# roahmlab/koopman-realizations

Hardware: AMD Instinct MI355X
Metric: EDMD snapshot-pairs/sec (bilinear fit, 3-link arm, poly-3) (higher is better)
Workload: dtype f64

## Files before the change

### koopman-realizations_amd/csrc/kp_context.hip

```cpp
#include <algorithm>
#include <cmath>
#include <cstring>
#include <mutex>

#include "kp_internal.h"

static std::mutex g_err_mu;
static std::string g_err;

void kp_set_global_error(const std::string& s) {
  std::lock_guard<std::mutex> l(g_err_mu);
  g_err = s;
}

void* kp_ctx::workspace(int slot, size_t bytes) {
  if (ws_bytes[slot] >= bytes && ws[slot]) return ws[slot];
  if (ws[slot]) (void)hipFree(ws[slot]);
  ws[slot] = nullptr;
  ws_bytes[slot] = 0;
  size_t want = bytes + bytes / 4 + 256;
  if (hipMalloc(&ws[slot], want) != hipSuccess) return nullptr;
  ws_bytes[slot] = want;
  return ws[slot];
}
// ... 50 lines not shown
  (void)kp_flush_grams(c);
  (void)kp_comm_destroy(c);
  (void)hipSetDevice(c->device);
  kp_stage_destroy(c);
  (void)hipStreamSynchronize(c->stream);
  if (c->stream2) (void)hipStreamSynchronize(c->stream2);
  for (int i = 0; i < 21; ++i)
    if (c->ws[i]) (void)hipFree(c->ws[i]);
  if (c->sticky_info) (void)hipFree(c->sticky_info);
  if (c->pin_small) (void)hipHostFree(c->pin_small);
  if (c->pin_scratch) (void)hipHostFree(c->pin_scratch);
  if (c->ev_gram_done) (void)hipEventDestroy(c->ev_gram_done);
  if (c->ev_pad_done) (void)hipEventDestroy(c->ev_pad_done);
  if (c->ev_pad_done2) (void)hipEventDestroy(c->ev_pad_done2);
  if (c->ev_main_done) (void)hipEventDestroy(c->ev_main_done);
  if (c->ev_solve0) (void)hipEventDestroy(c->ev_solve0);
  if (c->ev_solve1) (void)hipEventDestroy(c->ev_solve1);
  if (c->stream2) (void)hipStreamDestroy(c->stream2);
  if (c->Kres) (void)hipFree(c->Kres);
  if (c->GC) (void)hipFree(c->GC);
  for (int i = 0; i < 6; ++i)
    if (c->evp[i]) (void)hipEventDestroy(c->evp[i]);
  for (int i = 0; i < 2 * 64; ++i)
    if (c->ring[i]) (void)hipEventDestroy(c->ring[i]);
  for (int i = 0; i < 64; ++i)
    if (c->ring_red[i]) (void)hipEventDestroy(c->ring_red[i]);
  (void)hipEventDestroy(c->ev0);
  (void)hipEventDestroy(c->ev1);
  (void)hipStreamDestroy(c->stream);
  kp_traj_pool_free(c);
  kp_host_free_all(c);
  delete c;
  return KP_OK;
}

extern "C" int kp_device_count(int* count) {
  if (!count) return KP_ERR_ARG;
  int n = 0;
  if (hipGetDeviceCount(&n) != hipSuccess) {
    (void)hipGetLastError();
    n = 0;
  }
  *count = n;
  return KP_OK;
}

extern "C" const char* kp_last_error(const kp_ctx* c) {
  if (c) return c->err.c_str();
  std::lock_guard<std::mutex> l(g_err_mu);
  static thread_local std::string copy;
  copy = g_err;
  return copy.c_str();
}

extern "C" int kp_device_info(const kp_ctx* c, char* name, int name_len, int* num_cu, int64_t* hbm) {
  if (!c) return KP_ERR_ARG;
  if (name && name_len > 0) {
    std::strncpy(name, c->name.c_str(), (size_t)name_len - 1);
    name[name_len - 1] = 0;
  }
  if (num_cu) *num_cu = c->num_cu;
  if (hbm) *hbm = c->hbm_bytes;
  return KP_OK;
}

void* kp_pinned_scratch(kp_ctx* ctx, size_t bytes) {
  if (ctx->pin_scratch_bytes >= bytes) return ctx->pin_scratch;
  if (ctx->pin_scratch) {
    (void)hipStreamSynchronize(ctx->stream);
    (void)hipHostFree(ctx->pin_scratch);
  }
  ctx->pin_scratch = nullptr;
  ctx->pin_scratch_bytes = 0;
  const size_t cap = (bytes + 4095) & ~(size_t)4095;
  if (hipHostMalloc(&ctx->pin_scratch, cap, hipHostMallocDefault) != hipSuccess) {
    ctx->pin_scratch = nullptr;
    return nullptr;
  }
  ctx->pin_scratch_bytes = cap;
  return ctx->pin_scratch;
}

extern "C" int kp_timer_get(const kp_ctx* c, int which, double* ms) {
  if (!c || !ms || which < 0 || which >= 18) return KP_ERR_ARG;
  *ms = c->timers[which];
  return KP_OK;
}

extern "C" void* kp_stream(const kp_ctx* c) { return c ? (void*)c->stream : nullptr; }


static int upload(kp_ctx* ctx, void** dst, const void* src, size_t bytes) {
  *dst = nullptr;
  if (bytes == 0) return KP_OK;
  KP_HIP(ctx, hipMalloc(dst, bytes));
  KP_HIP(ctx, hipMemcpy(*dst, src, bytes, hipMemcpyHostToDevice));
  return KP_OK;
}

extern "C" int kp_basis_desc_dims(const kp_basis_desc* d, int* nvars_out, int* nfull_out, int* N_out, int* W_out) {
  if (!d || d->nzeta < 1 || d->m < 0 || d->model_type < 0 || d->model_type > 2 || d->n_blocks < 0 ||
      (d->n_blocks && (!d->block_type || !d->block_count)))
    return KP_ERR_ARG;
  const int nvars = d->nzeta + (d->model_type == KP_MODEL_NONLINEAR ? d->m : 0);
  double nf = nvars + 1.0;
  for (int b = 0; b < d->n_blocks; ++b) {
    const int c = d->block_count[b];
    if (c < 0) return KP_ERR_ARG;
    switch (d->block_type[b]) {
      case KP_BLOCK_POLY: case KP_BLOCK_HERMITE: case KP_BLOCK_FOURIER_SPARSER: case KP_BLOCK_GAUSSIAN: nf += c; break;
      case KP_BLOCK_FOURIER: nf += std::pow((double)(2 * c + 1), (double)nvars) - 1.0; break;
      default: return KP_ERR_ARG;
    }
    if (nf > 1e6) return KP_ERR_ARG;
  }
  const int nfull = (int)std::llround(nf);
  const int N = d->k_pcs > 0 ? d->k_pcs + nvars + 1 : nfull;
  if (nvars_out) *nvars_out = nvars;
  if (nfull_out) *nfull_out = nfull;
  if (N_out) *N_out = N;
  if (W_out) *W_out = d->model_type == KP_MODEL_BILINEAR ? N * (d->m + 1) : d->model_type == KP_MODEL_LINEAR ? N + d->m : N;
  return KP_OK;
}

extern "C" int kp_basis_create(kp_ctx* ctx, const kp_basis_desc* d, kp_basis** out) {
  if (!ctx || !d || !out) return KP_ERR_ARG;
  *out = nullptr;
  KP_HIP(ctx, hipSetDevice(ctx->device));
  if (d->model_type < 0 || d->model_type > 2) return ctx->fail(KP_ERR_ARG, "kp_basis_create: model_type");
  if (d->nzeta < 1 || d->m < 0) return ctx->fail(KP_ERR_ARG, "kp_basis_create: nzeta/m");
  int nvars = d->nzeta + (d->model_type == KP_MODEL_NONLINEAR ? d->m : 0);
  if (nvars > KP_MAX_VARS) return ctx->fail(KP_ERR_ARG, "kp_basis_create: too many variables (max 32)");
  std::vector<ColDesc> cols;
  for (int i = 0; i < nvars; ++i) cols.push_back({COL_VAR, i, 0, 0});
  int n_mono = 0, n_gauss = 0, max_deg = 1, fourier_deg = 0;
  for (int b = 0; b < d->n_blocks; ++b) {
    int cnt = d->block_count[b];
    if (cnt < 0) return ctx->fail(KP_ERR_ARG, "kp_basis_create: negative block count");
    switch (d->block_type[b]) {
      case KP_BLOCK_POLY:
        if (cnt && !d->poly_exps) return ctx->fail(KP_ERR_ARG, "kp_basis_create: poly_exps is NULL");
        for (int i = 0; i < cnt; ++i) {
          int deg = 0;
          for (int v = 0; v < nvars; ++v) deg += d->poly_exps[(size_t)(n_mono + i) * nvars + v];
          if (deg > max_deg) max_deg = deg;
          uint32_t pk[2] = {0, 0};
          if (nvars <= 8)
            for (int v = 0; v < nvars; ++v) pk[v >> 2] |= (uint32_t)d->poly_exps[(size_t)(n_mono + i) * nvars + v] << (8 * (v & 3));
          cols.push_back({COL_MONO, n_mono + i, (int32_t)pk[0], (int32_t)pk[1]});
        }
        n_mono += cnt;
        break;
      case KP_BLOCK_FOURIER: {
        if (cnt < 1) return ctx->fail(KP_ERR_ARG, "kp_basis_create: fourier degree < 1");
        double nf = std::pow((double)(2 * cnt + 1), (double)nvars);
        if (nf > 1e6) return ctx->fail(KP_ERR_ARG, "kp_basis_create: fourier block too large");
        int total = (int)std::llround(nf);
        for (int i = 1; i < total; ++i) {
          uint32_t pk = 0;
          if (nvars <= 8 && 2 * cnt + 1 <= 16) {
            int idx = i;
            for (int v = nvars - 1; v >= 0; --v) {
              pk |= (uint32_t)(idx % (2 * cnt + 1)) << (4 * v);
              idx /= 2 * cnt + 1;
            }
          }
          cols.push_back({COL_FOURIER, i, cnt, (int32_t)pk});
// ... 380 lines not shown
```

### koopman-realizations_amd/csrc/kp_fit.hip

```cpp
#include <cmath>
#include <cstdlib>

#include <vector>
#include <algorithm>
#include <cstring>

#include "kp_internal.h"

typedef double double4_t __attribute__((ext_vector_type(4)));
extern "C" int kp_synchronize(kp_ctx* ctx);

__global__ __launch_bounds__(256) void kp_pad_kernel(const double* __restrict__ G, const double* __restrict__ C, int W, int ncols, int n, int ncp,
                                                     double* __restrict__ Gp, double* __restrict__ Cp, size_t gc_stride) {
  const int i = blockIdx.x * 256 + threadIdx.x, jj = blockIdx.y;
  if (i >= n) return;
  G += blockIdx.z * gc_stride; C += blockIdx.z * gc_stride; Gp += blockIdx.z * (size_t)n * n; Cp += blockIdx.z * (size_t)n * ncp;
  if (jj < n) {
    Gp[(size_t)jj * n + i] = (i < W && jj < W) ? G[(size_t)jj * W + i] : (i == jj ? 1.0 : 0.0);
  } else {
    const int j = jj - n;
    Cp[(size_t)j * n + i] = (i < W && j < ncols) ? C[(size_t)j * W + i] : 0.0;
  }
}

__global__ __launch_bounds__(256) void kp_unpad_kernel(const double* __restrict__ Xp, int n, int W, int ncols, double* __restrict__ K, int ncp, int k_first, int k_cap) {
  const int i = blockIdx.x * 256 + threadIdx.x, j = blockIdx.y;
  if (i >= W) return;
  Xp += blockIdx.z * (size_t)n * ncp;
  if (k_cap > 0) K += (size_t)((k_first + (int)blockIdx.z) % k_cap) * W * ncols;
  K[(size_t)j * W + i] = Xp[(size_t)j * n + i];
}

#define PS 17

__device__ __forceinline__ double lane_bcast(double v, int lane) {
  int lo = __builtin_amdgcn_readlane(__double2loint(v), lane);
  int hi = __builtin_amdgcn_readlane(__double2hiint(v), lane);
  return __hiloint2double(hi, lo);
}

#define CH_NT 512

__device__ __forceinline__ void chol_diag_block(double* __restrict__ A, int n, int k0, double (*D)[16], double* Dd, int* bad,
                                                const double* __restrict__ odiag) {
  const int lane = threadIdx.x & 63;
  const int r = lane & 15;
  double row[16];
#pragma unroll
  for (int c = 0; c < 16; ++c) row[c] = A[(size_t)(k0 + c) * n + k0 + r];
#pragma unroll
  for (int c = 0; c < 16; ++c) {
    double d = lane_bcast(row[c], c);
    if (!(d > odiag[k0 + c])) {
      if (lane == 0) *bad = 1;
      d = 1.0;
    }
    double id = __builtin_amdgcn_rsq(d);
    id = id * (1.5 - 0.5 * d * id * id);
    id = id * (1.5 - 0.5 * d * id * id);
    if (lane == c) Dd[c] = id;
    const double l = row[c] * id;
    row[c] = l;
#pragma unroll
    for (int cc = c + 1; cc < 16; ++cc) row[cc] -= l * lane_bcast(l, cc);
  }
  if (lane < 16) {
#pragma unroll
    for (int c = 0; c < 16; ++c) {
      const double lrc = c <= r ? row[c] : 0.0;
      D[r][c] = lrc;
      if (c <= r) {
        A[(size_t)(k0 + c) * n + k0 + r] = lrc;
        A[(size_t)(k0 + r) * n + k0 + c] = lrc;
      }
    }
  }
}

__device__ __forceinline__ void chol_tile_update(double* __restrict__ A22, int n, const double* __restrict__ Lt, int ld, int ti, int tj,
                                                 double* __restrict__ Pnext) {
  double acc[8][8];
#pragma unroll
  for (int y = 0; y < 8; ++y) {
    const double2* src = reinterpret_cast<const double2*>(A22 + (size_t)(8 * tj + y) * n + 8 * ti);
#pragma unroll
    for (int h = 0; h < 4; ++h) {
      const double2 v = src[h];
      acc[2 * h][y] = v.x;
      acc[2 * h + 1][y] = v.y;
    }
// ... 159 lines not shown
                                                     double* __restrict__ X) {
  extern __shared__ double xs[];
  double* part = xs + (size_t)n * 16;
  const int tid = threadIdx.x, lane = tid & 63, wave = tid >> 6;
  const int cb = blockIdx.x;
  const int nt = n / 16;
  const int lr = lane >> 4, lc = lane & 15;
  LU += blockIdx.y * (size_t)n * n; Dinv += blockIdx.y * (size_t)nt * 256; X += blockIdx.y * (size_t)n * gridDim.x * 16;
  double* Xb = X + (size_t)cb * 16 * n;
  for (int e = tid; e < n * 16; e += 256) {
    int row = e % n, col = e / n;
    xs[row * 16 + col] = Xb[(size_t)col * n + row];
  }
  __syncthreads();
  double an[TR_MAXJ][4];
  for (int dir = 0; dir < 2; ++dir) {
    auto load_ops = [&](int i) {
#pragma unroll
      for (int s = 0; s < TR_MAXJ; ++s) {
        const int jj = wave + 4 * s;
        const int j = dir == 0 ? jj : nt - 1 - jj;
        const bool on = dir == 0 ? (j < i) : (j > i);
        if (i >= 0 && i < nt && on) {
#pragma unroll
          for (int kk = 0; kk < 4; ++kk) an[s][kk] = -LU[(size_t)(j * 16 + kk * 4 + lr) * n + i * 16 + lc];
        }
      }
    };
    const int i0 = dir == 0 ? 0 : nt - 1, istep = dir == 0 ? 1 : -1;
    load_ops(i0);
    for (int it = 0; it < nt; ++it) {
      const int i = i0 + it * istep;
      double ac[TR_MAXJ][4];
#pragma unroll
      for (int s = 0; s < TR_MAXJ; ++s)
#pragma unroll
        for (int kk = 0; kk < 4; ++kk) ac[s][kk] = an[s][kk];
      load_ops(i + istep);
      double4_t acc = {0.0, 0.0, 0.0, 0.0};
#pragma unroll
      for (int s = 0; s < TR_MAXJ; ++s) {
        const int jj = wave + 4 * s;
        const int j = dir == 0 ? jj : nt - 1 - jj;
        const bool on = dir == 0 ? (j < i) : (j > i);
        if (on) {
#pragma unroll
          for (int kk = 0; kk < 4; ++kk) {
            const double bv = xs[(j * 16 + kk * 4 + lr) * 16 + lc];
            acc = __builtin_amdgcn_mfma_f64_16x16x4f64(ac[s][kk], bv, acc, 0, 0, 0);
          }
        }
      }
#pragma unroll
      for (int r = 0; r < 4; ++r) part[wave * 256 + (lr + 4 * r) * 16 + lc] = acc[r];
      __syncthreads();
      if (wave == 0) {
        double4_t y = {0.0, 0.0, 0.0, 0.0};
#pragma unroll
        for (int kk = 0; kk < 4; ++kk) {
          const int k = kk * 4 + lr;
          const double av = dir == 0 ? Dinv[(size_t)i * 256 + k * 16 + lc] : Dinv[(size_t)i * 256 + lc * 16 + k];
          const int o = k * 16 + lc;
          const double bv = xs[(i * 16 + k) * 16 + lc] + part[o] + part[256 + o] + part[512 + o] + part[768 + o];
          y = __builtin_amdgcn_mfma_f64_16x16x4f64(av, bv, y, 0, 0, 0);
        }
#pragma unroll
        for (int r = 0; r < 4; ++r) xs[(i * 16 + lr + 4 * r) * 16 + lc] = y[r];
      }
      __syncthreads();
    }
  }
  for (int e = tid; e < n * 16; e += 256) {
    int row = e % n, col = e / n;
    Xb[(size_t)col * n + row] = xs[row * 16 + col];
  }
}

static bool trsm_old_sel() {
  static const bool v = getenv("KP_TRSM_OLD") != nullptr;
  return v;
}

#define TR2_MAXR 8
namespace {

template <int NJ>
__device__ __forceinline__ int tr2_col(int c) { return (c & 3) * NJ + (c >> 2); }

template <int CNT>
__device__ __forceinline__ void tr2_load(double (&an)[TR2_MAXR][4], const double* __restrict__ LU, int64_t n, int jc, const int (&rowof)[TR2_MAXR], int kq,
                                         int blk, int jj) {
#pragma unroll
  for (int q = 0; q < CNT; ++q)
#pragma unroll
    for (int K = 0; K < 4; ++K) an[q][K] = -LU[(size_t)(jc * 16 + 4 * K + kq) * n + rowof[q] * 16 + 4 * blk + jj];
}

template <int CNT, int NJ>
__device__ __forceinline__ void tr2_update(double (&acc)[TR2_MAXR][NJ], const double (&an)[TR2_MAXR][4], const double (&bv)[4][NJ], int q0) {
#pragma unroll
  for (int q = 0; q < CNT; ++q) {
    if (q < q0) continue;
#pragma unroll
    for (int K = 0; K < 4; ++K)
#pragma unroll
      for (int J = 0; J < NJ; ++J) acc[q][J] = __builtin_amdgcn_mfma_f64_4x4x4f64(an[q][K], bv[K][J], acc[q][J], 0, 0, 0);
  }
}

template <int NJ>
__device__ __forceinline__ void tr2_get(const double* __restrict__ xs, int row, int jj, double (&v)[NJ]) {
  const double* p = xs + row * (4 * NJ) + jj * NJ;
  if constexpr (NJ == 4) {
    const double2 v01 = reinterpret_cast<const double2*>(p)[0], v23 = reinterpret_cast<const double2*>(p)[1];
    v[0] = v01.x; v[1] = v01.y; v[2] = v23.x; v[3] = v23.y;
  } else if constexpr (NJ == 2) {
    const double2 v01 = reinterpret_cast<const double2*>(p)[0];
    v[0] = v01.x; v[1] = v01.y;
  } else {
    v[0] = p[0];
  }
}

template <int NJ>
__device__ __forceinline__ void tr2_put(double* __restrict__ xs, int row, int jj, const double (&v)[NJ]) {
  double* p = xs + row * (4 * NJ) + jj * NJ;
  if constexpr (NJ == 4) {
    double2 v01, v23;
    v01.x = v[0]; v01.y = v[1]; v23.x = v[2]; v23.y = v[3];
    reinterpret_cast<double2*>(p)[0] = v01; reinterpret_cast<double2*>(p)[1] = v23;
  } else if constexpr (NJ == 2) {
    double2 v01;
    v01.x = v[0]; v01.y = v[1];
    reinterpret_cast<double2*>(p)[0] = v01;
  } else {
    p[0] = v[0];
  }
}

template <int NJ>
__device__ __forceinline__ void tr2_read_b(const double* __restrict__ xs, int j, int kq, int jj, double (&b)[4][NJ]) {
#pragma unroll
  for (int K = 0; K < 4; ++K) tr2_get<NJ>(xs, j * 16 + 4 * K + kq, jj, b[K]);
}

}

#define TR2_SWITCH(CALL)                                                                   \
  switch (cnt) {                                                                           \
    case 1: { constexpr int C_ = 1; CALL; } break;                                         \
    case 2: { constexpr int C_ = 2; CALL; } break;                                         \
    case 3: { constexpr int C_ = 3; CALL; } break;                                         \
    case 4: { constexpr int C_ = 4; CALL; } break;                                         \
    case 5: { constexpr int C_ = 5; CALL; } break;                                         \
    case 6: { constexpr int C_ = 6; CALL; } break;                                         \
    case 7: { constexpr int C_ = 7; CALL; } break;                                         \
    case 8: { constexpr int C_ = 8; CALL; } break;                                         \
    default: break;                                                                        \
  }

template <int NJ>
__global__ __launch_bounds__(256) void kp_trsm2_kernel(const double* __restrict__ LU, const double* __restrict__ Dinv, int n, int ncp,
                                                      double* __restrict__ X, double* __restrict__ Kout, int W, int ncols, int64_t ldl, int64_t ldx,
                                                      int dirs, const int* __restrict__ info) {
  if (info && info[blockIdx.y]) return;
  extern __shared__ __align__(16) double xs[];
  constexpr int NC = 4 * NJ;
  const int tid = threadIdx.x, lane = tid & 63;
  const int wave = __builtin_amdgcn_readfirstlane(tid >> 6);
  const int cb = blockIdx.x;
  const int nt = n / 16;
  const int kq = lane >> 4, blk = (lane >> 2) & 3, jj = lane & 3;
  LU += blockIdx.y * (size_t)n * n; Dinv += blockIdx.y * (size_t)nt * 256; X += blockIdx.y * (size_t)ldx * ncp;
  double* Xb = X + (size_t)cb * NC * ldx;
  for (int e = tid; e < n * NC; e += 256) {
    int row = e % n, col = e / n;
    xs[row * NC + tr2_col<NJ>(col)] = Xb[(size_t)col * ldx + row];
  }
  __syncthreads();
  const int nown = wave < nt ? (nt - wave + 3) / 4 : 0;
  for (int dir = 0; dir < 2; ++dir) {
    if (!((dirs >> dir) & 1)) continue;
    int rowof[TR2_MAXR];
#pragma unroll
    for (int q = 0; q < TR2_MAXR; ++q) rowof[q] = q < nown ? (dir == 0 ? wave + 4 * (nown - 1 - q) : wave + 4 * q) : 0;
    double acc[TR2_MAXR][NJ];
#pragma unroll
    for (int q = 0; q < TR2_MAXR; ++q) tr2_get<NJ>(xs, rowof[q] * 16 + 4 * blk + kq, jj, acc[q]);
    auto beyond = [&](int j) {
      const int c = dir == 0 ? nown - (j < wave ? 0 : (j - wave) / 4 + 1) : (j <= wave ? 0 : (j - wave + 3) / 4);
      return min(max(c, 0), nown);
    };
    const int j0 = dir == 0 ? 0 : nt - 1, jstep = dir == 0 ? 1 : -1;
    auto load_dinv = [&](int j, double (&dv)[4]) {
      const int jc = min(max(j, 0), nt - 1);
#pragma unroll
      for (int K = 0; K < 4; ++K) {
        const int r = 4 * blk + jj, c = 4 * K + kq;
        dv[K] = dir == 0 ? Dinv[(size_t)jc * 256 + c * 16 + r] : Dinv[(size_t)jc * 256 + r * 16 + c];
      }
    };
    double dv[4];
    {
      int jf = j0;
      while (jf >= 0 && jf < nt && (jf & 3) != wave) jf += jstep;
      load_dinv(jf, dv);
    }
    double an[TR2_MAXR][4];
    double bv[4][NJ];
    int cnt = nown;
    for (int it = 0; it < nt; ++it) {
      const int j = j0 + it * jstep;
      const bool owner = (j & 3) == wave;
      if (owner) {
        const int qj = cnt - 1;
        if (it > 0) { TR2_SWITCH((tr2_update<C_, NJ>(acc, an, bv, C_ - 1))); }
        double rj[NJ];
#pragma unroll
        for (int J = 0; J < NJ; ++J) rj[J] = acc[0][J];
#pragma unroll
        for (int q = 1; q < TR2_MAXR; ++q)
          if (q == qj) {
#pragma unroll
            for (int J = 0; J < NJ; ++J) rj[J] = acc[q][J];
          }
        tr2_put<NJ>(xs, j * 16 + 4 * blk + kq, jj, rj);
        __builtin_amdgcn_fence(__ATOMIC_RELEASE, "wavefront");
        __builtin_amdgcn_wave_barrier();
        __builtin_amdgcn_fence(__ATOMIC_ACQUIRE, "wavefront");
        double br[4][NJ];
        tr2_read_b<NJ>(xs, j, kq, jj, br);
        double y[NJ];
#pragma unroll
        for (int J = 0; J < NJ; ++J) y[J] = 0.0;
#pragma unroll
        for (int K = 0; K < 4; ++K)
#pragma unroll
          for (int J = 0; J < NJ; ++J) y[J] = __builtin_amdgcn_mfma_f64_4x4x4f64(dv[K], br[K][J], y[J], 0, 0, 0);
        __builtin_amdgcn_fence(__ATOMIC_RELEASE, "wavefront");
        __builtin_amdgcn_wave_barrier();
        __builtin_amdgcn_fence(__ATOMIC_ACQUIRE, "wavefront");
        tr2_put<NJ>(xs, j * 16 + 4 * blk + kq, jj, y);
        load_dinv(j + 4 * jstep, dv);
        if (it > 0) { TR2_SWITCH((tr2_update<C_ - 1, NJ>(acc, an, bv, 0))); }
      } else if (it > 0) {
        TR2_SWITCH((tr2_update<C_, NJ>(acc, an, bv, 0)));
      }
      cnt = beyond(j);
      TR2_SWITCH((tr2_load<C_>(an, LU, ldl, j, rowof, kq, blk, jj)));
      asm volatile("s_waitcnt lgkmcnt(0)\n\ts_barrier" ::: "memory");
      tr2_read_b<NJ>(xs, j, kq, jj, bv);
    }
    __syncthreads();
  }
  for (int e = tid; e < n * NC; e += 256) {
    int row = e % n, col = e / n;
    const double v = xs[row * NC + tr2_col<NJ>(col)];
    if (Kout) {
      const int gc = cb * NC + col;
      if (row < W && gc < ncols) Kout[(size_t)gc * W + row] = v;
    } else {
      Xb[(size_t)col * ldx + row] = v;
    }
  }
}

__global__ __launch_bounds__(256) void kp_wide_thresh_kernel(const double* __restrict__ A, int n, double* __restrict__ thr) {
  const int i = blockIdx.x * 256 + threadIdx.x;
  if (i < n) thr[i] = fmax(A[(size_t)i * n + i], 0.0) * ((double)n * 8.0 * 2.220446049250313e-16);
}

__global__ __launch_bounds__(256) void kp_wide_diag_kernel(double* __restrict__ A, int n, int k0, int b, double* __restrict__ D, int back) {
  const int e = blockIdx.x * 256 + threadIdx.x;
  if (e >= b * b) return;
  const int i = e % b, j = e / b;
  if (back) A[(size_t)(k0 + j) * n + k0 + i] = D[e];
  else D[e] = A[(size_t)(k0 + max(i, j)) * n + k0 + min(i, j)];
}

static int wide_block() {
  const char* e = getenv("KP_WIDE_BS");
  const int b = e ? atoi(e) : 256;
  return std::max(16, std::min(352, b)) / 16 * 16;
}

#include "kp_tn_gemm.h"

static hipError_t wide_trsm(hipStream_t st, const double* Akk, const double* Dinv_k, int b, int nrhs, double* X, int n, int dirs) {
  if (nrhs <= 4096)
    hipLaunchKernelGGL((kp_trsm2_kernel<1>), dim3(nrhs / 4, 1), dim3(256), (size_t)b * 4 * 8, st, Akk, Dinv_k, b, nrhs, X, (double*)nullptr, 0, 0, (int64_t)n, (int64_t)n,
                       dirs, (const int*)nullptr);
  else
    hipLaunchKernelGGL((kp_trsm2_kernel<4>), dim3(nrhs / 16, 1), dim3(256), (size_t)b * 16 * 8, st, Akk, Dinv_k, b, nrhs, X, (double*)nullptr, 0, 0, (int64_t)n, (int64_t)n,
                       dirs, (const int*)nullptr);
  return hipGetLastError();
}

static int wide_substitute(kp_ctx* ctx, double* Gp, double* Cp, double* Dinv, int n, int ncp, hipStream_t st, bool forward_done = false) {
  const int bs = wide_block();
  static KpLdsCache trsm_lds;
  KP_HIP(ctx, kp_ensure_lds(trsm_lds, (const void*)kp_trsm2_kernel<4>, (size_t)352 * 16 * 8));
  for (int k0 = 0; k0 < n && !forward_done; k0 += bs) {
    const int b = std::min(bs, n - k0), R = n - k0 - b;
    KP_HIP(ctx, wide_trsm(st, Gp + (size_t)k0 * n + k0, Dinv + (size_t)(k0 / 16) * 256, b, ncp, Cp + k0, n, 1));
    if (R > 0) KP_HIP(ctx, kp_tn_gemm(st, Gp + (size_t)(k0 + b) * n + k0, n, Cp + k0, n, R, ncp, b, Cp + k0 + b, n, -1.0, 1.0, 0, 1, nullptr));
  }
  for (int k0 = (n - 1) / bs * bs; k0 >= 0; k0 -= bs) {
    const int b = std::min(bs, n - k0);
    KP_HIP(ctx, wide_trsm(st, Gp + (size_t)k0 * n + k0, Dinv + (size_t)(k0 / 16) * 256, b, ncp, Cp + k0, n, 2));
    if (k0 > 0) KP_HIP(ctx, kp_tn_gemm(st, Gp + k0, n, Cp + k0, n, k0, ncp, b, Cp, n, -1.0, 1.0, 0, 1, nullptr));
  }
  return KP_OK;
}

static int chol_solve_wide(kp_ctx* ctx, double* Gp, double* Cp, double* Dinv, int n, int ncp, int* info, int* sticky, hipStream_t st) {
  const int bs = wide_block();
  double* scr = (double*)ctx->workspace(18, ((size_t)bs * bs + n) * 8 + 64);
  if (!scr) return ctx->fail(KP_ERR_HIP, "kp_fit_solve: out of device memory");
  double* D = scr;
  double* thr = scr + (size_t)bs * bs;
  int* dummy = (int*)(thr + n);
  static KpLdsCache trsm_lds;
  KP_HIP(ctx, kp_ensure_lds(trsm_lds, (const void*)kp_trsm2_kernel<4>, (size_t)352 * 16 * 8));
  const bool fwd = Cp == Gp + (size_t)n * n && !getenv("KP_WIDE_SEPARATE_FORWARD");
  KP_HIP(ctx, hipMemsetAsync(info, 0, sizeof(int), st));
  hipLaunchKernelGGL(kp_wide_thresh_kernel, dim3((n + 255) / 256), dim3(256), 0, st, Gp, n, thr);
  for (int k0 = 0; k0 < n; k0 += bs) {
    const int b = std::min(bs, n - k0), R = n - k0 - b;
    double* Akk = Gp + (size_t)k0 * n + k0;
    double* A12 = Gp + (size_t)(k0 + b) * n + k0;
    hipLaunchKernelGGL(kp_wide_diag_kernel, dim3((b * b + 255) / 256), dim3(256), 0, st, Gp, n, k0, b, D, 0);
    KP_HIP(ctx, kp_chol_ll_launch(D, b, 1, dummy, info, 0, st, thr + k0));
    {
      const int nbk = b / 16, npair = nbk * (nbk - 1) / 2;
      hipLaunchKernelGGL(kp_chol_finish_kernel, dim3(npair + nbk, 1), dim3(256), 0, st, D, b, npair, Dinv + (size_t)(k0 / 16) * 256);
    }
    hipLaunchKernelGGL(kp_wide_diag_kernel, dim3((b * b + 255) / 256), dim3(256), 0, st, Gp, n, k0, b, D, 1);
    KP_HIP(ctx, hipGetLastError());
    if (fwd) {
      KP_HIP(ctx, wide_trsm(st, Akk, Dinv + (size_t)(k0 / 16) * 256, b, R + ncp, A12, n, 1));
      if (R > 0) KP_HIP(ctx, kp_tn_gemm(st, A12, n, A12, n, R, R + ncp, b, Gp + (size_t)(k0 + b) * n + k0 + b, n, -1.0, 1.0, 1, 1, nullptr));
    } else if (R > 0) {
      KP_HIP(ctx, wide_trsm(st, Akk, Dinv + (size_t)(k0 / 16) * 256, b, R, A12, n, 1));
      KP_HIP(ctx, kp_tn_gemm(st, A12, n, A12, n, R, R, b, Gp + (size_t)(k0 + b) * n + k0 + b, n, -1.0, 1.0, 1, 1, nullptr));
    }
  }
  hipLaunchKernelGGL(kp_mirror_upper_kernel, dim3(n / 16, n / 16), dim3(256), 0, st, Gp, n, (int64_t)n);
  KP_HIP(ctx, hipGetLastError());
  if (sticky) {
    KP_HIP(ctx, hipMemcpyAsync(sticky, info, sizeof(int), hipMemcpyDeviceToDevice, st));
  }
  return wide_substitute(ctx, Gp, Cp, Dinv, n, ncp, st, fwd);
}

int kp_factor_substitute_dev(kp_ctx* ctx, double* Lp, int n, double* Cp, int ncp, double* Dinv, hipStream_t st, int* form) {
  if (!st) st = ctx->stream;
  const int nbk = n / 16, npair = nbk * (nbk - 1) / 2;
  hipLaunchKernelGGL(kp_chol_finish_kernel, dim3(npair + nbk, 1), dim3(256), 0, st, Lp, n, npair, Dinv);
  KP_HIP(ctx, hipGetLastError());
  if (form) *form = n > 16 * 4 * TR_MAXJ ? 3 : ncp <= 512 ? 1 : 2;
  if (n > 16 * 4 * TR_MAXJ) return wide_substitute(ctx, Lp, Cp, Dinv, n, ncp, st);
  static KpLdsCache trsm2_lds;
  KP_HIP(ctx, kp_ensure_lds(trsm2_lds, (const void*)kp_trsm2_kernel<4>, (size_t)352 * 16 * 8 > (size_t)n * 16 * 8 ? (size_t)352 * 16 * 8 : (size_t)n * 16 * 8));
  if (ncp <= 512)
    hipLaunchKernelGGL((kp_trsm2_kernel<1>), dim3(ncp / 4, 1), dim3(256), (size_t)n * 4 * 8, st, Lp, Dinv, n, ncp, Cp, (double*)nullptr, 0, 0, (int64_t)n, (int64_t)n, 3, (const int*)nullptr);
  else
    hipLaunchKernelGGL((kp_trsm2_kernel<4>), dim3(ncp / 16, 1), dim3(256), (size_t)n * 16 * 8, st, Lp, Dinv, n, ncp, Cp, (double*)nullptr, 0, 0, (int64_t)n, (int64_t)n, 3, (const int*)nullptr);
  KP_HIP(ctx, hipGetLastError());
  return KP_OK;
}

int kp_chol_solve_batch_dev(kp_ctx* ctx, const double* G_dev, const double* C_dev, int W, int ncols, int nb, size_t gc_stride, double* K_dev,
                            int k_first, int k_cap, hipStream_t st, hipEvent_t pad_done, int* sticky) {
  if (!st) st = ctx->stream;
  const int n = (W + 15) / 16 * 16, ncp = (ncols + 15) / 16 * 16;
  size_t bG = (size_t)n * n * 8, bC = (size_t)n * ncp * 8, bD = (size_t)(n / 16) * 256 * 8;
  char* ws = (char*)ctx->workspace(5, (size_t)nb * (bG + bC + bD) + (size_t)nb * 4 + 64);
  if (!ws) return ctx->fail(KP_ERR_HIP, "kp_fit_solve: out of device memory");
  double* Gp = (double*)ws;
  double* Cp = (double*)(ws + (size_t)nb * bG);
  double* Dinv = (double*)(ws + (size_t)nb * (bG + bC));
  int* info = (int*)(ws + (size_t)nb * (bG + bC + bD));
  size_t lds_chol = (size_t)2 * 16 * n * 8;
  size_t lds_trsm = ((size_t)n * 16 + 1024) * 8;
  const bool wide = n > 16 * 4 * TR_MAXJ;
  if (wide && nb != 1) return ctx->fail(KP_ERR_ARG, "kp_fit_solve: systems wider than 512 are solved one at a time");
  if (!wide && (lds_chol > 160 * 1024 - 8192 || lds_trsm > 160 * 1024)) return ctx->fail(KP_ERR_ARG, "kp_fit_solve: W too large");
  hipLaunchKernelGGL(kp_pad_kernel, dim3((n + 255) / 256, n + ncp, nb), dim3(256), 0, st, G_dev, C_dev, W, ncols, n, ncp, Gp, Cp, gc_stride);
  KP_HIP(ctx, hipGetLastError());
  if (pad_done) KP_HIP(ctx, hipEventRecord(pad_done, st));
  if (wide) {
    int rc = chol_solve_wide(ctx, Gp, Cp, Dinv, n, ncp, info, sticky, st);
    if (rc) return rc;
    double* Kdst = K_dev + (k_cap > 0 ? (size_t)(k_first % k_cap) * W * ncols : 0);
    hipLaunchKernelGGL(kp_unpad_kernel, dim3((W + 255) / 256, ncols, 1), dim3(256), 0, st, Cp, n, W, ncols, Kdst, ncp, 0, 0);
    KP_HIP(ctx, hipGetLastError());
    return KP_OK;
  }
  static KpLdsCache chol_lds, trsm_lds;
  static const int chol_prof = getenv("KP_CHOL_PROF") ? atoi(getenv("KP_CHOL_PROF")) : 0;
  if (kp_chol_ll_applicable(n)) {
    KP_HIP(ctx, kp_chol_ll_launch(Gp, n, nb, info, sticky, chol_prof, st));
  } else {
    KP_HIP(ctx, kp_ensure_lds(chol_lds, (const void*)kp_chol_kernel, lds_chol));
    hipLaunchKernelGGL(kp_chol_kernel, dim3(1, nb), dim3(CH_NT), lds_chol, st, Gp, n, Dinv, info, sticky, chol_prof);
    KP_HIP(ctx, hipGetLastError());
  }
  {
    const int nbk = n / 16, npair = nbk * (nbk - 1) / 2;
    hipLaunchKernelGGL(kp_chol_finish_kernel, dim3(npair + nbk, nb), dim3(256), 0, st, Gp, n, npair, Dinv);
  }
  KP_HIP(ctx, hipGetLastError());
  if (trsm_old_sel()) {
    KP_HIP(ctx, kp_ensure_lds(trsm_lds, (const void*)kp_trsm_kernel, lds_trsm));
    hipLaunchKernelGGL(kp_trsm_kernel, dim3(ncp / 16, nb), dim3(256), lds_trsm, st, Gp, Dinv, n, Cp);
  } else if (nb == 1) {
    double* Kdst = K_dev + (k_cap > 0 ? (size_t)(k_first % k_cap) * W * ncols : 0);
    hipLaunchKernelGGL((kp_trsm2_kernel<1>), dim3(ncp / 4, nb), dim3(256), (size_t)n * 4 * 8, st, Gp, Dinv, n, ncp, Cp, Kdst, W, ncols, (int64_t)n,
                       (int64_t)n, 3, (const int*)info);
    KP_HIP(ctx, hipGetLastError());
    return KP_OK;
  } else {
    static KpLdsCache trsm2_lds;
    KP_HIP(ctx, kp_ensure_lds(trsm2_lds, (const void*)kp_trsm2_kernel<4>, (size_t)n * 16 * 8));
    hipLaunchKernelGGL((kp_trsm2_kernel<4>), dim3(ncp / 16, nb), dim3(256), (size_t)n * 16 * 8, st, Gp, Dinv, n, ncp, Cp, (double*)nullptr, W, ncols,
                       (int64_t)n, (int64_t)n, 3, (const int*)info);
  }
  KP_HIP(ctx, hipGetLastError());
  hipLaunchKernelGGL(kp_unpad_kernel, dim3((W + 255) / 256, ncols, nb), dim3(256), 0, st, Cp, n, W, ncols, K_dev, ncp, k_first,
                     k_cap);
  KP_HIP(ctx, hipGetLastError());
  return KP_OK;
}

int kp_chol_solve_dev(kp_ctx* ctx, double* G_dev, double* C_dev, int W, int ncols, double* K_dev, hipStream_t st, hipEvent_t pad_done,
                      int* sticky) {
  return kp_chol_solve_batch_dev(ctx, G_dev, C_dev, W, ncols, 1, 0, K_dev, 0, 0, st, pad_done, sticky);
}

__global__ __launch_bounds__(256) void kp_pivot_ratio_kernel(const double* __restrict__ Lp, int n, const double* __restrict__ G, int W,
                                                             double* __restrict__ out, const int* __restrict__ info, double* host_out) {
  __shared__ double red[4];
  double r = 1e300;
  for (int i = threadIdx.x; i < W; i += 256) {
    const double l = Lp[(size_t)i * n + i], g = G[(size_t)i * W + i];
    r = fmin(r, g > 0.0 ? l * l / g : 0.0);
  }
#pragma unroll
  for (int o = 32; o > 0; o >>= 1) r = fmin(r, __shfl_xor(r, o, 64));
  if ((threadIdx.x & 63) == 0) red[threadIdx.x >> 6] = r;
  __syncthreads();
  if (threadIdx.x == 0) {
    const double v = fmin(fmin(red[0], red[1]), fmin(red[2], red[3]));
    out[0] = v;
    if (host_out) {
      host_out[1] = v;
      *reinterpret_cast<int*>(host_out) = info[0];
      __threadfence_system();
    }
  }
}

static int check_info(kp_ctx* ctx) {
  return KP_OK;
}

static int read_chol_info(kp_ctx* ctx, int W, int ncols, int* bad, const double* G_dev = nullptr, hipStream_t st = nullptr, int phase = 0) {
  if (!st) st = ctx->stream;
  const int n = (W + 15) / 16 * 16;
  const size_t off = kp_chol_info_offset(W, ncols);
  double* ratio_dev = (double*)((char*)ctx->ws[5] + off + 8);
  if (G_dev && phase != 2) {
    hipLaunchKernelGGL(kp_pivot_ratio_kernel, dim3(1), dim3(256), 0, st, (const double*)ctx->ws[5], n, G_dev, W, ratio_dev,
                       (const int*)((char*)ctx->ws[5] + off), ctx->pin_small);
    KP_HIP(ctx, hipGetLastError());
  }
  if (phase == 1) return KP_OK;
  if (ctx->pin_small) {
    if (!G_dev) KP_HIP(ctx, hipMemcpyAsync(ctx->pin_small, (char*)ctx->ws[5] + off, 16, hipMemcpyDeviceToHost, st));
    KP_HIP(ctx, hipStreamSynchronize(st));
    int info = 0;
    memcpy(&info, ctx->pin_small, sizeof(int));
    *bad = info;
    if (G_dev) ctx->last_pivot_ratio = ctx->pin_small[1];
  } else {
    if (G_dev) KP_HIP(ctx, hipMemcpyAsync(&ctx->last_pivot_ratio, ratio_dev, sizeof(double), hipMemcpyDeviceToHost, st));
    KP_HIP(ctx, hipMemcpyAsync(bad, (char*)ctx->ws[5] + off, sizeof(int), hipMemcpyDeviceToHost, st));
    KP_HIP(ctx, hipStreamSynchronize(st));
  }
  (void)check_info;
  return KP_OK;
}

static void collect_gram_timers(kp_ctx* ctx, bool solved) {
  float ms = 0;
  bool red_done = false;
  if (ctx->ring_n > 0) {
    double sum = 0.0, rsum = 0.0;
    int cnt = 0, fits = 0, rfits = 0;
    for (int i = 0; i < ctx->ring_n; ++i) {
      const int p = (ctx->ring_pos - 1 - i + 2 * 64) % 64;
      if (hipEventElapsedTime(&ms, ctx->ring[2 * p], ctx->ring[2 * p + 1]) == hipSuccess) {
// ... 501 lines not shown
```

### koopman-realizations_amd/csrc/kp_internal.h

```cpp
#pragma once
#include <hip/hip_runtime.h>
#include <stdint.h>
#include <atomic>
#include <mutex>
#include <string>
#include <utility>
#include <vector>

#include "koopman_hip.h"

#define KP_MAX_VARS 32
#define KP_GRAM_GROUP_MAX 8

void kp_set_global_error(const std::string& s);
void kp_traj_device_blocks(kp_traj* t, double** blocks);
struct kp_comm_state;

struct kp_stage;

struct kp_ctx {
  int device = 0;
  kp_stage* stage = nullptr;
  std::vector<void*> host_blocks;
  std::vector<std::pair<void*, size_t>> traj_pool;
  std::mutex host_mu;
  hipStream_t stream = nullptr;
  hipEvent_t ev0 = nullptr, ev1 = nullptr;
  hipEvent_t evp[6] = {nullptr};
  hipStream_t stream2 = nullptr;
  hipEvent_t ev_gram_done = nullptr, ev_pad_done = nullptr, ev_pad_done2 = nullptr, ev_solve0 = nullptr, ev_solve1 = nullptr;
  bool pad_pending = false, pad_pending2 = false, async_pending = false;
  int gc_flip = 0;
  int kring_cap = 128;
  int async_count = 0;
  bool batch_closed = true;
  bool kres_is_ring = false;
  const void* pend_basis = nullptr;
  int64_t pend_Ns = 0;
  int pend_W = 0;
  int pend_solves = 0, pend_first = 0;
  bool ring_timing = false;
  unsigned ring_skip = 0;
  const kp_snapshots* pend_grams[KP_GRAM_GROUP_MAX] = {};
  int pend_ngrams = 0;
  const kp_basis* pend_gram_basis = nullptr;
  double* pend_gram_gc = nullptr;
  bool ring_group = false;
  kp_comm_state* comm = nullptr;
  std::atomic<bool> comm_abandoned{false};
  bool gc_preloaded = false;
  bool reduce_grams = false;
  hipStream_t reduce_stream = nullptr;
  hipEvent_t ev_main_done = nullptr;
  hipEvent_t ring[2 * 64] = {};
  int ring_pos = 0, ring_n = 0;
  hipEvent_t ring_red[64] = {};
  int ring_members[64] = {};
  bool ring_has_red[64] = {};
  bool solve_chained = false;
  int part_flip = 0;
  int reduce_timed_from = 1;
  int* sticky_info = nullptr;
  bool test_hooks = false;
  void* pin_scratch = nullptr;
  size_t pin_scratch_bytes = 0;
  double* pin_small = nullptr;
  int reserve_cus = 0;
  int num_cu = 0;
  int64_t hbm_bytes = 0;
  std::string name;
  mutable std::string err;
  double timers[18] = {0};
  double gram_flops_per_pair = 0;
  void* ws[21] = {nullptr};
  size_t ws_bytes[21] = {0};
  int last_rank = -1;
  double last_pivot_ratio = 1.0;
  double* Kres = nullptr;
  size_t Kres_bytes = 0;
  int Kres_W = 0, Kres_n = 0;
  double* GC = nullptr;
  size_t GC_bytes = 0;
  int GC_W = 0;

  int fail(int code, const std::string& s) const {
    err = s;
    kp_set_global_error(s);
    return code;
  }
  void* workspace(int slot, size_t bytes);
};

#define KP_HIP(ctx, expr)                                                                  \
  do {                                                                                     \
    hipError_t _e = (expr);                                                                \
    if (_e != hipSuccess)                                                                  \
      return (ctx)->fail(KP_ERR_HIP, std::string(#expr) + ": " + hipGetErrorString(_e));   \
  } while (0)

enum : int { COL_VAR = 0, COL_MONO = 1, COL_FOURIER = 2, COL_GAUSS = 3, COL_CONST = 4, COL_HERMITE = 5, COL_FSPARSE = 6 };

struct ColDesc {
  int32_t kind;
  int32_t arg;
  int32_t aux;
  int32_t pad;
};

struct BasisDev {
  int model_type, nzeta, m, nvars;
  int nfull, N, W, k_pcs;
  const ColDesc* cols;
  const uint8_t* exps;
  const double* centres;
  const double* pcs;
};

struct KpLdsCache { size_t set[32] = {}; };
inline hipError_t kp_ensure_lds(KpLdsCache& c, const void* func, size_t lds) {
  int dev = -1;
  if (hipGetDevice(&dev) != hipSuccess || dev < 0 || dev >= 32) return hipFuncSetAttribute(func, hipFuncAttributeMaxDynamicSharedMemorySize, (int)lds);
  if (lds > c.set[dev]) {
    hipError_t e = hipFuncSetAttribute(func, hipFuncAttributeMaxDynamicSharedMemorySize, (int)lds);
    if (e != hipSuccess) return e;
    c.set[dev] = lds;
  }
  return hipSuccess;
}

struct kp_gram_plan;
void kp_gram_plan_free(kp_gram_plan* p);
struct kp_gram2_plan;
void kp_gram2_plan_free(kp_gram2_plan* p);
struct kp_gram3_plan;
void kp_gram3_plan_free(kp_gram3_plan* p);
struct kp_gram5_plan;
void kp_gram5_plan_free(kp_gram5_plan* p);

struct kp_basis {
  kp_ctx* ctx = nullptr;
  BasisDev dev{};
  void* d_cols = nullptr;
  void* d_exps = nullptr;
  void* d_centres = nullptr;
  void* d_pcs = nullptr;
  void* d_recipes = nullptr;
  void* d_pcsT = nullptr;
  int max_degree = 0;
  mutable int rank_hint = 0;
  bool pure_fourier = false;
  int fourier_degree = 0;
  int pow_depth = 1;
  bool fast = false;
  int max_factors = 1;
  kp_gram_plan* plan = nullptr;
// ... 179 lines not shown
```

Before: 328.8 million.

## Add batched triangular-solve kernel reading C directly with XCD-aware block mapping

For batched small systems, a new batch trsm kernel reads the unpadded right-hand side C directly and writes K straight to the output ring. This removes padding of C and the separate unpad kernel launch. Blocks are remapped so all column blocks of one system land on the same XCD for L2 locality, the kernel uses a smaller register budget (max 6 row tiles, launch bounds with 2 blocks per CU), and singular systems copy C through. A diagnostic timer slot records which path ran.

```diff
diff --git a/koopman-realizations_amd/csrc/kp_context.hip b/koopman-realizations_amd/csrc/kp_context.hip
--- a/koopman-realizations_amd/csrc/kp_context.hip
+++ b/koopman-realizations_amd/csrc/kp_context.hip
@@ -156,7 +156,7 @@
 }
 
 extern "C" int kp_timer_get(const kp_ctx* c, int which, double* ms) {
-  if (!c || !ms || which < 0 || which >= 18) return KP_ERR_ARG;
+  if (!c || !ms || which < 0 || which >= 19) return KP_ERR_ARG;
   *ms = c->timers[which];
   return KP_OK;
 }
diff --git a/koopman-realizations_amd/csrc/kp_fit.hip b/koopman-realizations_amd/csrc/kp_fit.hip
--- a/koopman-realizations_amd/csrc/kp_fit.hip
+++ b/koopman-realizations_amd/csrc/kp_fit.hip
@@ -6,6 +6,7 @@
 #include <cstring>
 
 #include "kp_internal.h"
+#include "kp_solve_xcd_map.h"
 
 typedef double double4_t __attribute__((ext_vector_type(4)));
 extern "C" int kp_synchronize(kp_ctx* ctx);
@@ -331,13 +332,14 @@
 }
 
 #define TR2_MAXR 8
+#define TR2_BATCH_MAXR 6
 namespace {
 
 template <int NJ>
 __device__ __forceinline__ int tr2_col(int c) { return (c & 3) * NJ + (c >> 2); }
 
-template <int CNT>
-__device__ __forceinline__ void tr2_load(double (&an)[TR2_MAXR][4], const double* __restrict__ LU, int64_t n, int jc, const int (&rowof)[TR2_MAXR], int kq,
+template <int CNT, int MAXR>
+__device__ __forceinline__ void tr2_load(double (&an)[MAXR][4], const double* __restrict__ LU, int64_t n, int jc, const int (&rowof)[MAXR], int kq,
                                          int blk, int jj) {
 #pragma unroll
   for (int q = 0; q < CNT; ++q)
@@ -345,8 +347,8 @@
     for (int K = 0; K < 4; ++K) an[q][K] = -LU[(size_t)(jc * 16 + 4 * K + kq) * n + rowof[q] * 16 + 4 * blk + jj];
 }
 
-template <int CNT, int NJ>
-__device__ __forceinline__ void tr2_update(double (&acc)[TR2_MAXR][NJ], const double (&an)[TR2_MAXR][4], const double (&bv)[4][NJ], int q0) {
+template <int CNT, int NJ, int MAXR>
+__device__ __forceinline__ void tr2_update(double (&acc)[MAXR][NJ], const double (&an)[MAXR][4], const double (&bv)[4][NJ], int q0) {
 #pragma unroll
   for (int q = 0; q < CNT; ++q) {
     if (q < q0) continue;
@@ -403,39 +405,44 @@
     case 4: { constexpr int C_ = 4; CALL; } break;                                         \
     case 5: { constexpr int C_ = 5; CALL; } break;                                         \
     case 6: { constexpr int C_ = 6; CALL; } break;                                         \
-    case 7: { constexpr int C_ = 7; CALL; } break;                                         \
-    case 8: { constexpr int C_ = 8; CALL; } break;                                         \
+    case 7: if constexpr (MAXR >= 7) { constexpr int C_ = 7; CALL; } break;                \
+    case 8: if constexpr (MAXR >= 8) { constexpr int C_ = 8; CALL; } break;                \
     default: break;                                                                        \
   }
 
-template <int NJ>
-__global__ __launch_bounds__(256) void kp_trsm2_kernel(const double* __restrict__ LU, const double* __restrict__ Dinv, int n, int ncp,
-                                                      double* __restrict__ X, double* __restrict__ Kout, int W, int ncols, int64_t ldl, int64_t ldx,
-                                                      int dirs, const int* __restrict__ info) {
-  if (info && info[blockIdx.y]) return;
+template <int NJ, int MAXR, bool RING>
+__device__ __forceinline__ void tr2_body(const double* __restrict__ LU, const double* __restrict__ Dinv, int n, double* __restrict__ X,
+                                         const double* __restrict__ Cin, double* __restrict__ Kout, int W, int ncols, int64_t ldl, int64_t ldx, int dirs,
+                                         int cb) {
   extern __shared__ __align__(16) double xs[];
   constexpr int NC = 4 * NJ;
   const int tid = threadIdx.x, lane = tid & 63;
   const int wave = __builtin_amdgcn_readfirstlane(tid >> 6);
-  const int cb = blockIdx.x;
   const int nt = n / 16;
   const int kq = lane >> 4, blk = (lane >> 2) & 3, jj = lane & 3;
-  LU += blockIdx.y * (size_t)n * n; Dinv += blockIdx.y * (size_t)nt * 256; X += blockIdx.y * (size_t)ldx * ncp;
-  double* Xb = X + (size_t)cb * NC * ldx;
+  double* Xb = nullptr;
+  if constexpr (!RING) Xb = X + (size_t)cb * NC * ldx;
   for (int e = tid; e < n * NC; e += 256) {
     int row = e % n, col = e / n;
-    xs[row * NC + tr2_col<NJ>(col)] = Xb[(size_t)col * ldx + row];
+    double v;
+    if constexpr (RING) {
+      const int gc = cb * NC + col;
+      v = (row < W && gc < ncols) ? Cin[(size_t)gc * W + row] : 0.0;
+    } else {
+      v = Xb[(size_t)col * ldx + row];
+    }
+    xs[row * NC + tr2_col<NJ>(col)] = v;
   }
   __syncthreads();
   const int nown = wave < nt ? (nt - wave + 3) / 4 : 0;
   for (int dir = 0; dir < 2; ++dir) {
     if (!((dirs >> dir) & 1)) continue;
-    int rowof[TR2_MAXR];
-#pragma unroll
-    for (int q = 0; q < TR2_MAXR; ++q) rowof[q] = q < nown ? (dir == 0 ? wave + 4 * (nown - 1 - q) : wave + 4 * q) : 0;
-    double acc[TR2_MAXR][NJ];
-#pragma unroll
-    for (int q = 0; q < TR2_MAXR; ++q) tr2_get<NJ>(xs, rowof[q] * 16 + 4 * blk + kq, jj, acc[q]);
+    int rowof[MAXR];
+#pragma unroll
+    for (int q = 0; q < MAXR; ++q) rowof[q] = q < nown ? (dir == 0 ? wave + 4 * (nown - 1 - q) : wave + 4 * q) : 0;
+    double acc[MAXR][NJ];
+#pragma unroll
+    for (int q = 0; q < MAXR; ++q) tr2_get<NJ>(xs, rowof[q] * 16 + 4 * blk + kq, jj, acc[q]);
     auto beyond = [&](int j) {
       const int c = dir == 0 ? nown - (j < wave ? 0 : (j - wave) / 4 + 1) : (j <= wave ? 0 : (j - wave + 3) / 4);
       return min(max(c, 0), nown);
@@ -455,7 +462,7 @@
       while (jf >= 0 && jf < nt && (jf & 3) != wave) jf += jstep;
       load_dinv(jf, dv);
     }
-    double an[TR2_MAXR][4];
+    double an[MAXR][4];
     double bv[4][NJ];
     int cnt = nown;
     for (int it = 0; it < nt; ++it) {
@@ -463,12 +470,12 @@
       const bool owner = (j & 3) == wave;
       if (owner) {
         const int qj = cnt - 1;
-        if (it > 0) { TR2_SWITCH((tr2_update<C_, NJ>(acc, an, bv, C_ - 1))); }
+        if (it > 0) { TR2_SWITCH((tr2_update<C_, NJ, MAXR>(acc, an, bv, C_ - 1))); }
         double rj[NJ];
 #pragma unroll
         for (int J = 0; J < NJ; ++J) rj[J] = acc[0][J];
 #pragma unroll
-        for (int q = 1; q < TR2_MAXR; ++q)
+        for (int q = 1; q < MAXR; ++q)
           if (q == qj) {
 #pragma unroll
             for (int J = 0; J < NJ; ++J) rj[J] = acc[q][J];
@@ -491,12 +498,12 @@
         __builtin_amdgcn_fence(__ATOMIC_ACQUIRE, "wavefront");
         tr2_put<NJ>(xs, j * 16 + 4 * blk + kq, jj, y);
         load_dinv(j + 4 * jstep, dv);
-        if (it > 0) { TR2_SWITCH((tr2_update<C_ - 1, NJ>(acc, an, bv, 0))); }
+        if (it > 0) { TR2_SWITCH((tr2_update<C_ - 1, NJ, MAXR>(acc, an, bv, 0))); }
       } else if (it > 0) {
-        TR2_SWITCH((tr2_update<C_, NJ>(acc, an, bv, 0)));
+        TR2_SWITCH((tr2_update<C_, NJ, MAXR>(acc, an, bv, 0)));
       }
       cnt = beyond(j);
-      TR2_SWITCH((tr2_load<C_>(an, LU, ldl, j, rowof, kq, blk, jj)));
+      TR2_SWITCH((tr2_load<C_, MAXR>(an, LU, ldl, j, rowof, kq, blk, jj)));
       asm volatile("s_waitcnt lgkmcnt(0)\n\ts_barrier" ::: "memory");
       tr2_read_b<NJ>(xs, j, kq, jj, bv);
     }
@@ -505,13 +512,41 @@
   for (int e = tid; e < n * NC; e += 256) {
     int row = e % n, col = e / n;
     const double v = xs[row * NC + tr2_col<NJ>(col)];
-    if (Kout) {
+    if (RING || Kout) {
       const int gc = cb * NC + col;
       if (row < W && gc < ncols) Kout[(size_t)gc * W + row] = v;
     } else {
       Xb[(size_t)col * ldx + row] = v;
     }
   }
+}
+
+template <int NJ>
+__global__ __launch_bounds__(256) void kp_trsm2_kernel(const double* __restrict__ LU, const double* __restrict__ Dinv, int n, int ncp,
+                                                      double* __restrict__ X, double* __restrict__ Kout, int W, int ncols, int64_t ldl, int64_t ldx,
+                                                      int dirs, const int* __restrict__ info) {
+  if (info && info[blockIdx.y]) return;
+  const int nt = n / 16;
+  LU += blockIdx.y * (size_t)n * n; Dinv += blockIdx.y * (size_t)nt * 256; X += blockIdx.y * (size_t)ldx * ncp;
+  tr2_body<NJ, TR2_MAXR, false>(LU, Dinv, n, X, (const double*)nullptr, Kout, W, ncols, ldl, ldx, dirs, (int)blockIdx.x);
+}
+
+__global__ __launch_bounds__(256, 2) void kp_trsm2_batch_kernel(const double* __restrict__ LU, const double* __restrict__ Dinv, int n, int ncp, int nb,
+                                                                const double* __restrict__ C, size_t gc_stride, double* __restrict__ K, int W,
+                                                                int ncols, int k_first, int k_cap, const int* __restrict__ info) {
+  int sys, cb;
+  if (!kp_solve_xcd_map(blockIdx.x, ncp / 16, nb, &sys, &cb)) return;
+  C += sys * gc_stride;
+  if (k_cap > 0) K += (size_t)((k_first + sys) % k_cap) * W * ncols;
+  if (info[sys]) {
+    for (int e = threadIdx.x; e < W * 16; e += 256) {
+      const int row = e % W, gc = cb * 16 + e / W;
+      if (gc < ncols) K[(size_t)gc * W + row] = C[(size_t)gc * W + row];
+    }
+    return;
+  }
+  const int nt = n / 16;
+  tr2_body<4, TR2_BATCH_MAXR, true>(LU + sys * (size_t)n * n, Dinv + sys * (size_t)nt * 256, n, (double*)nullptr, C, K, W, ncols, (int64_t)n, (int64_t)n, 3, cb);
 }
 
 __global__ __launch_bounds__(256) void kp_wide_thresh_kernel(const double* __restrict__ A, int n, double* __restrict__ thr) {
@@ -619,6 +654,11 @@
   return KP_OK;
 }
 
+static bool solve_batch_form_new() {
+  static const bool v = [] { const char* e = getenv("KP_SOLVE_BATCH_FORM"); return !e || atoi(e) != 0; }();
+  return v;
+}
+
 int kp_chol_solve_batch_dev(kp_ctx* ctx, const double* G_dev, const double* C_dev, int W, int ncols, int nb, size_t gc_stride, double* K_dev,
                             int k_first, int k_cap, hipStream_t st, hipEvent_t pad_done, int* sticky) {
   if (!st) st = ctx->stream;
@@ -635,7 +675,9 @@
   const bool wide = n > 16 * 4 * TR_MAXJ;
   if (wide && nb != 1) return ctx->fail(KP_ERR_ARG, "kp_fit_solve: systems wider than 512 are solved one at a time");
   if (!wide && (lds_chol > 160 * 1024 - 8192 || lds_trsm > 160 * 1024)) return ctx->fail(KP_ERR_ARG, "kp_fit_solve: W too large");
-  hipLaunchKernelGGL(kp_pad_kernel, dim3((n + 255) / 256, n + ncp, nb), dim3(256), 0, st, G_dev, C_dev, W, ncols, n, ncp, Gp, Cp, gc_stride);
+  const bool batch_entry = nb > 1 && !wide && n <= 16 * 4 * TR2_BATCH_MAXR && solve_batch_form_new() && !trsm_old_sel();
+  if (nb > 1) ctx->timers[18] = batch_entry ? 211.0 : 100.0;
+  hipLaunchKernelGGL(kp_pad_kernel, dim3((n + 255) / 256, batch_entry ? n : n + ncp, nb), dim3(256), 0, st, G_dev, C_dev, W, ncols, n, ncp, Gp, Cp, gc_stride);
   KP_HIP(ctx, hipGetLastError());
   if (pad_done) KP_HIP(ctx, hipEventRecord(pad_done, st));
   if (wide) {
@@ -667,6 +709,13 @@
     double* Kdst = K_dev + (k_cap > 0 ? (size_t)(k_first % k_cap) * W * ncols : 0);
     hipLaunchKernelGGL((kp_trsm2_kernel<1>), dim3(ncp / 4, nb), dim3(256), (size_t)n * 4 * 8, st, Gp, Dinv, n, ncp, Cp, Kdst, W, ncols, (int64_t)n,
                        (int64_t)n, 3, (const int*)info);
+    KP_HIP(ctx, hipGetLastError());
+    return KP_OK;
+  } else if (batch_entry) {
+    static KpLdsCache batch_lds;
+    KP_HIP(ctx, kp_ensure_lds(batch_lds, (const void*)kp_trsm2_batch_kernel, (size_t)n * 16 * 8));
+    hipLaunchKernelGGL(kp_trsm2_batch_kernel, dim3(kp_solve_xcd_grid(ncp / 16, nb)), dim3(256), (size_t)n * 16 * 8, st, Gp, Dinv, n, ncp, nb, C_dev, gc_stride,
+                       K_dev, W, ncols, k_first, k_cap, (const int*)info);
     KP_HIP(ctx, hipGetLastError());
     return KP_OK;
   } else {
diff --git a/koopman-realizations_amd/csrc/kp_internal.h b/koopman-realizations_amd/csrc/kp_internal.h
--- a/koopman-realizations_amd/csrc/kp_internal.h
+++ b/koopman-realizations_amd/csrc/kp_internal.h
@@ -70,7 +70,7 @@
   int64_t hbm_bytes = 0;
   std::string name;
   mutable std::string err;
-  double timers[18] = {0};
+  double timers[19] = {0};
   double gram_flops_per_pair = 0;
   void* ws[21] = {nullptr};
   size_t ws_bytes[21] = {0};
diff --git a/koopman-realizations_amd/csrc/kp_solve_xcd_map.h b/koopman-realizations_amd/csrc/kp_solve_xcd_map.h
--- /dev/null
+++ b/koopman-realizations_amd/csrc/kp_solve_xcd_map.h
@@ -0,0 +1,20 @@
+#pragma once
+
+#if defined(__HIPCC__) || defined(__CUDACC__)
+#define KP_XCD_HD __host__ __device__
+#else
+#define KP_XCD_HD
+#endif
+
+#define KP_SOLVE_XCDS 8
+
+KP_XCD_HD inline unsigned kp_solve_xcd_grid(int ncb, int nb) {
+  return (unsigned)ncb * KP_SOLVE_XCDS * (unsigned)((nb + KP_SOLVE_XCDS - 1) / KP_SOLVE_XCDS);
+}
+
+KP_XCD_HD inline bool kp_solve_xcd_map(unsigned id, int ncb, int nb, int* system, int* cb) {
+  const unsigned k = id / KP_SOLVE_XCDS;
+  *system = (int)(k / (unsigned)ncb) * KP_SOLVE_XCDS + (int)(id % KP_SOLVE_XCDS);
+  *cb = (int)(k % (unsigned)ncb);
+  return *system < nb;
+}
```

New measurement: 334.0 million (median of 6 runs). 1.02x the previous value.
